# vnoz/Mutual-Information-MultiModal

Hardware: AMD Instinct MI355X
Metric: img-txt pairs/sec (MI critic fwd+bwd), global-batch InfoNCE (higher is better)
Workload: dtype bf16; 1 GPU; BASELINE configs[3]: global-batch infonce (reference semantics), bilinear critic fwd+bwd, B_global=4096, d=512; global_batch=4096, embed_dim=512, critic=bilinear, estimator=infonce, parallelism=single GPU, boundary=fp32 embeddings in, fp32 gradients out, hip_graph=False, graph_mode=none (direct C-ABI calls)

## Files before the change

mutual-information-multimodal_amd/csrc/mi_bilinear_flash.h:

```cpp
#pragma once
#include <type_traits>

#include "mi_common.h"

namespace mi {

#ifdef MI_STAMPS
#define MI_FL_STAMP(slot)                                                                       \
  do {                                                                                          \
    __builtin_amdgcn_sched_barrier(0);                                                          \
    if (threadIdx.x == 0 && g_stamps) g_stamps[(size_t)blockIdx.x * 16 + (slot)] = __builtin_amdgcn_s_memtime(); \
    __builtin_amdgcn_sched_barrier(0);                                                          \
  } while (0)
#else
#define MI_FL_STAMP(slot) do {} while (0)
#endif

#ifndef MI_FL_DIAG
#define MI_FL_DIAG 0
#endif
constexpr int kFlDiag = MI_FL_DIAG;
constexpr int kFlRows = 128;
constexpr int kFlBN = 32;
constexpr int kFlStages = 4;
constexpr float kFlThr = 60.0f;
constexpr int kFlMaxTilesPerSplit = 64;

struct FlashProblem {
  const bf16_t* q;
  const bf16_t* kv;
  const int64_t* sid_q;
  const int64_t* sid_kv;
  int64_t m, n;
  int64_t diag;
  int n_rb;
  int n_split;
  int tiles_per_split;
  const unsigned char* dup;
  float* slab;
  Partial* rec;
};
struct FlashArgs {
  FlashProblem p[2];
  int n_problems;
  int n_combo;
  int xcd_rows;
  int diag;
  int slab_f16;
  int no_index_mask;
};

template <int D>
struct FlashCfg {
  static constexpr int NK = D / 16;
  static constexpr int NT = D / 32;
  static constexpr int RB = D * 2;
  static constexpr int CPR = RB / 16;
  static constexpr int RPP = 1024 / RB;
  static constexpr int STAGE = kFlBN * RB;
  static constexpr int PIECES = STAGE / 1024 / 4;
  static constexpr int SID_OFF = kFlStages * STAGE;
  static constexpr size_t SMEM = (size_t)SID_OFF + (size_t)kFlMaxTilesPerSplit * kFlBN * 8;
  static constexpr int QA = NT >= 16 ? NK / 2 : 0;
  static constexpr int OA = NT >= 16 ? 12 : NT;
  static_assert(D == 128 || D == 256 || D == 512, "unsupported embedding width");
};

__host__ __device__ constexpr int fl_swz(int row) { return ((row & 3) << 2) | ((row >> 2) & 3); }

__device__ __forceinline__ float wave_max_uniform(float v) {
  int x;
#define MI_DPP_MAX(ctrl, rmask)                                                        \
  x = __builtin_amdgcn_update_dpp(__float_as_int(v), __float_as_int(v), ctrl, rmask, 0xF, false); \
  v = fmaxf(v, __int_as_float(x));
  MI_DPP_MAX(0xB1, 0xF)
  MI_DPP_MAX(0x4E, 0xF)
  MI_DPP_MAX(0x141, 0xF)
  MI_DPP_MAX(0x140, 0xF)
  MI_DPP_MAX(0x142, 0xA)
  MI_DPP_MAX(0x143, 0xC)
#undef MI_DPP_MAX
  return __int_as_float(__builtin_amdgcn_readlane(__float_as_int(v), 63));
}

__device__ __forceinline__ void fl_dma16(unsigned voff, const void* sbase, unsigned lds_addr) {
  unsigned keep;
  const uintptr_t b = (uintptr_t)sbase;
  const unsigned blo = __builtin_amdgcn_readfirstlane((unsigned)b), bhi = __builtin_amdgcn_readfirstlane((unsigned)(b >> 32));
  sbase = (const void*)(((uintptr_t)bhi << 32) | blo);
  lds_addr = __builtin_amdgcn_readfirstlane(lds_addr);
  asm volatile("s_mov_b32 %0, m0\n\ts_mov_b32 m0, %3\n\ts_nop 1\n\tglobal_load_lds_dwordx4 %1, %2\n\ts_mov_b32 m0, %0"
               : "=&s"(keep)
               : "v"(voff), "s"(sbase), "s"(lds_addr)
               : "memory");
}

template <int LOFF>
__device__ __forceinline__ void fl_dma_set_m0(unsigned lds_base) {
  asm volatile("s_add_u32 m0, %0, %1" : : "s"(lds_base), "n"(LOFF) : "scc");
}
template <int GOFF, int XORC>
__device__ __forceinline__ void fl_dma16_at(unsigned vlane_w, const void* sbase) {
  unsigned voff;
  asm volatile("v_xor_b32 %0, %3, %1\n\tglobal_load_lds_dwordx4 %0, %2 offset:%4"
               : "=&v"(voff)
               : "v"(vlane_w), "s"(sbase), "n"(XORC), "n"(GOFF)
               : "memory");
}

__device__ __forceinline__ float fl_max3(float a, float b, float c) {
  float d;
  asm("v_max3_f32 %0, %1, %2, %3" : "=v"(d) : "v"(a), "v"(b), "v"(c));
  return d;
}

__device__ __forceinline__ void fl_v_exp(const float& x) { asm volatile("v_exp_f32 %0, %0" : : "v"(x)); }
__device__ __forceinline__ void fl_v_add(const float& acc, const float& p) { asm volatile("v_add_f32 %0, %0, %1" : : "v"(acc), "v"(p)); }
__device__ __forceinline__ void fl_v_opaque(float& x) { asm volatile("; fl_opaque" : "+v"(x)); }
__device__ __forceinline__ unsigned fl_v_cvt_pk(const float& lo, const float& hi) {
  unsigned d;
  asm volatile("v_cvt_pk_bf16_f32 %0, %1, %2" : "=v"(d) : "v"(lo), "v"(hi));
  return d;
}
__device__ __forceinline__ void fl_v_prescale(float& x, const float& s, const float& off) {
  asm volatile("v_fmamk_f32 %0, %1, 0x3fb8aa3b, %2" : "=v"(x) : "v"(s), "v"(off));
}
__device__ __forceinline__ void fl_v_max(float& d, const float& a, const float& b) {
  asm volatile("v_max_f32 %0, %1, %2" : "=v"(d) : "v"(a), "v"(b));
}
__device__ __forceinline__ void fl_v_max3(float& d, const float& a, const float& b) {
  asm volatile("v_max3_f32 %0, %0, %1, %2" : "+v"(d) : "v"(a), "v"(b));
}
template <int STEP, bool NOP>
__device__ __forceinline__ void fl_dpp_max(const float& v) {
#define MI_FL_DPP(ctrl)                                                                            \
  if constexpr (NOP) asm volatile("s_nop 1\n\tv_max_f32_dpp %0, %0, %0 " ctrl : : "v"(v));          \
  else asm volatile("v_max_f32_dpp %0, %0, %0 " ctrl : : "v"(v))
  if constexpr (STEP == 0) { MI_FL_DPP("quad_perm:[1,0,3,2] row_mask:0xf bank_mask:0xf"); }
  else if constexpr (STEP == 1) { MI_FL_DPP("quad_perm:[2,3,0,1] row_mask:0xf bank_mask:0xf"); }
  else if constexpr (STEP == 2) { MI_FL_DPP("row_half_mirror row_mask:0xf bank_mask:0xf"); }
  else if constexpr (STEP == 3) { MI_FL_DPP("row_mirror row_mask:0xf bank_mask:0xf"); }
  else if constexpr (STEP == 4) { MI_FL_DPP("row_bcast:15 row_mask:0xa bank_mask:0xf"); }
  else { MI_FL_DPP("row_bcast:31 row_mask:0xc bank_mask:0xf"); }
#undef MI_FL_DPP
}

template <int N>
__device__ __forceinline__ void fl_wait_vmcnt_barrier() {
  asm volatile("s_waitcnt vmcnt(%0)\n\ts_barrier" ::"n"(N) : "memory");
}

template <int B, int E, class F>
__device__ __forceinline__ void fl_static_for(F&& f) {
  if constexpr (B < E) {
    f(std::integral_constant<int, B>{});
    fl_static_for<B + 1, E>(f);
  }
}

constexpr int kFlRing = 9;
constexpr int kFlAhead = 8;

template <int SLOT, int OFF>
__device__ __forceinline__ void fl_ring_read_s(bf16x8& f, int addr) {
  static_assert(OFF >= 0 && OFF < 65536, "ds offset field");
  if constexpr (SLOT == 0)
    asm volatile("ds_read_b128 v[216:219], %1 offset:%c2" : "={v[216:219]}"(f) : "v"(addr), "i"(OFF));
  else if constexpr (SLOT == 1)
    asm volatile("ds_read_b128 v[220:223], %1 offset:%c2" : "={v[220:223]}"(f) : "v"(addr), "i"(OFF));
  else if constexpr (SLOT == 2)
    asm volatile("ds_read_b128 v[224:227], %1 offset:%c2" : "={v[224:227]}"(f) : "v"(addr), "i"(OFF));
  else if constexpr (SLOT == 3)
    asm volatile("ds_read_b128 v[228:231], %1 offset:%c2" : "={v[228:231]}"(f) : "v"(addr), "i"(OFF));
  else if constexpr (SLOT == 4)
    asm volatile("ds_read_b128 v[232:235], %1 offset:%c2" : "={v[232:235]}"(f) : "v"(addr), "i"(OFF));
  else if constexpr (SLOT == 5)
    asm volatile("ds_read_b128 v[236:239], %1 offset:%c2" : "={v[236:239]}"(f) : "v"(addr), "i"(OFF));
  else if constexpr (SLOT == 6)
    asm volatile("ds_read_b128 v[240:243], %1 offset:%c2" : "={v[240:243]}"(f) : "v"(addr), "i"(OFF));
  else if constexpr (SLOT == 7)
    asm volatile("ds_read_b128 v[244:247], %1 offset:%c2" : "={v[244:247]}"(f) : "v"(addr), "i"(OFF));
  else if constexpr (SLOT == 8)
    asm volatile("ds_read_b128 v[248:251], %1 offset:%c2" : "={v[248:251]}"(f) : "v"(addr), "i"(OFF));
  else if constexpr (SLOT == 9)
    asm volatile("ds_read_b128 v[252:255], %1 offset:%c2" : "={v[252:255]}"(f) : "v"(addr), "i"(OFF));
}
template <int SLOT, int OFF_LO, int OFF_HI>
__device__ __forceinline__ void fl_ring_read_v(bf16x8& f, int addr_lo, int addr_hi) {
  static_assert(OFF_LO >= 0 && OFF_HI < 65536, "ds offset field");
  if constexpr (SLOT == 0)
    asm volatile("ds_read_b64_tr_b16 v[216:217], %1 offset:%c3\n\tds_read_b64_tr_b16 v[218:219], %2 offset:%c4"
                 : "={v[216:219]}"(f) : "v"(addr_lo), "v"(addr_hi), "i"(OFF_LO), "i"(OFF_HI));
  else if constexpr (SLOT == 1)
    asm volatile("ds_read_b64_tr_b16 v[220:221], %1 offset:%c3\n\tds_read_b64_tr_b16 v[222:223], %2 offset:%c4"
                 : "={v[220:223]}"(f) : "v"(addr_lo), "v"(addr_hi), "i"(OFF_LO), "i"(OFF_HI));
  else if constexpr (SLOT == 2)
    asm volatile("ds_read_b64_tr_b16 v[224:225], %1 offset:%c3\n\tds_read_b64_tr_b16 v[226:227], %2 offset:%c4"
                 : "={v[224:227]}"(f) : "v"(addr_lo), "v"(addr_hi), "i"(OFF_LO), "i"(OFF_HI));
  else if constexpr (SLOT == 3)
    asm volatile("ds_read_b64_tr_b16 v[228:229], %1 offset:%c3\n\tds_read_b64_tr_b16 v[230:231], %2 offset:%c4"
                 : "={v[228:231]}"(f) : "v"(addr_lo), "v"(addr_hi), "i"(OFF_LO), "i"(OFF_HI));
  else if constexpr (SLOT == 4)
    asm volatile("ds_read_b64_tr_b16 v[232:233], %1 offset:%c3\n\tds_read_b64_tr_b16 v[234:235], %2 offset:%c4"
                 : "={v[232:235]}"(f) : "v"(addr_lo), "v"(addr_hi), "i"(OFF_LO), "i"(OFF_HI));
  else if constexpr (SLOT == 5)
    asm volatile("ds_read_b64_tr_b16 v[236:237], %1 offset:%c3\n\tds_read_b64_tr_b16 v[238:239], %2 offset:%c4"
                 : "={v[236:239]}"(f) : "v"(addr_lo), "v"(addr_hi), "i"(OFF_LO), "i"(OFF_HI));
  else if constexpr (SLOT == 6)
    asm volatile("ds_read_b64_tr_b16 v[240:241], %1 offset:%c3\n\tds_read_b64_tr_b16 v[242:243], %2 offset:%c4"
                 : "={v[240:243]}"(f) : "v"(addr_lo), "v"(addr_hi), "i"(OFF_LO), "i"(OFF_HI));
  else if constexpr (SLOT == 7)
    asm volatile("ds_read_b64_tr_b16 v[244:245], %1 offset:%c3\n\tds_read_b64_tr_b16 v[246:247], %2 offset:%c4"
                 : "={v[244:247]}"(f) : "v"(addr_lo), "v"(addr_hi), "i"(OFF_LO), "i"(OFF_HI));
  else if constexpr (SLOT == 8)
    asm volatile("ds_read_b64_tr_b16 v[248:249], %1 offset:%c3\n\tds_read_b64_tr_b16 v[250:251], %2 offset:%c4"
                 : "={v[248:251]}"(f) : "v"(addr_lo), "v"(addr_hi), "i"(OFF_LO), "i"(OFF_HI));
  else if constexpr (SLOT == 9)
    asm volatile("ds_read_b64_tr_b16 v[252:253], %1 offset:%c3\n\tds_read_b64_tr_b16 v[254:255], %2 offset:%c4"
                 : "={v[252:255]}"(f) : "v"(addr_lo), "v"(addr_hi), "i"(OFF_LO), "i"(OFF_HI));
}
template <int WAIT>
__device__ __forceinline__ void fl_wait_lgkm() {
  if constexpr (kFlDiag & 16) return;
  if constexpr (WAIT >= 0) asm volatile("s_waitcnt lgkmcnt(%c0)" ::"i"(WAIT) : "memory");
}
template <bool B_IN_ACC, bool FIRST, int WAIT>
__device__ __forceinline__ void fl_mfma_s(f32x16& acc, const bf16x8& a, const bf16x8& b) {
  fl_wait_lgkm<WAIT>();
  if constexpr (FIRST) {
    if constexpr (B_IN_ACC)
      asm volatile("v_mfma_f32_32x32x16_bf16 %0, %1, %2, 0" : "=v"(acc) : "v"(a), "a"(b));
    else
      asm volatile("v_mfma_f32_32x32x16_bf16 %0, %1, %2, 0" : "=v"(acc) : "v"(a), "v"(b));
  } else {
    if constexpr (B_IN_ACC)
      asm volatile("v_mfma_f32_32x32x16_bf16 %0, %1, %2, %0" : : "v"(acc), "v"(a), "a"(b));
    else
      asm volatile("v_mfma_f32_32x32x16_bf16 %0, %1, %2, %0" : : "v"(acc), "v"(a), "v"(b));
  }
}
template <bool ACC_IN_ACC, bool NOP, int WAIT, class AT>
__device__ __forceinline__ void fl_mfma_o(f32x16& acc, const AT& a, const bf16x8& b) {
  static_assert(sizeof(AT) == 16, "a 32x32x16 bf16 operand is four registers");
  fl_wait_lgkm<WAIT>();
  if constexpr (NOP) {
    if constexpr (ACC_IN_ACC)
      asm volatile("s_nop 1\n\tv_mfma_f32_32x32x16_bf16 %0, %1, %2, %0" : "+a"(acc) : "v"(a), "v"(b));
    else
      asm volatile("s_nop 1\n\tv_mfma_f32_32x32x16_bf16 %0, %1, %2, %0" : "+v"(acc) : "v"(a), "v"(b));
  } else {
    if constexpr (ACC_IN_ACC)
      asm volatile("v_mfma_f32_32x32x16_bf16 %0, %1, %2, %0" : "+a"(acc) : "v"(a), "v"(b));
    else
      asm volatile("v_mfma_f32_32x32x16_bf16 %0, %1, %2, %0" : "+v"(acc) : "v"(a), "v"(b));
  }
}
template <bool DRAIN>
__device__ __forceinline__ void fl_score_fence(f32x16& acc) {
  if constexpr (DRAIN) asm volatile("s_nop 15\n\ts_nop 3" : "+v"(acc));
  else asm volatile("" : "+v"(acc));
}
__device__ __forceinline__ void fl_mfma_drain_all() { asm volatile("s_nop 15\n\ts_nop 3" ::: "memory"); }
template <bool IN_ACC>
__device__ __forceinline__ void fl_scale_tile(f32x16& t, float f) {
#pragma unroll
  for (int r = 0; r < 16; ++r) {
    if constexpr (IN_ACC) {
      float e = t[r], tmp;
      asm volatile("v_accvgpr_read_b32 %1, %0\n\tv_mul_f32 %1, %1, %2\n\tv_accvgpr_write_b32 %0, %1"
                   : "+a"(e), "=&v"(tmp)
                   : "v"(f));
      t[r] = e;
    } else {
      t[r] *= f;
    }
  }
}
template <bool IN_ACC>
__device__ __forceinline__ void fl_pin(bf16x8& v) {
  if constexpr (IN_ACC) asm volatile("" : "+a"(v));
  else asm volatile("" : "+v"(v));
}
template <bool IN_ACC>
__device__ __forceinline__ void fl_pin_o(f32x16& v) {
  if constexpr (IN_ACC) asm volatile("" : "+a"(v));
  else asm volatile("" : "+v"(v));
}

#ifndef MI_FL_WAIT_GROUP
#define MI_FL_WAIT_GROUP 2
#endif
constexpr int kFlWaitGroup = MI_FL_WAIT_GROUP;
template <int NS, int NV>
constexpr int fl_wait_count(int n) {
  if (n % kFlWaitGroup) return -1;
  int c = 0;
  for (int m = n + kFlWaitGroup; m <= n + kFlAhead - 1 && m < NS + NV; ++m) c += m < NS ? 1 : 2;
  return c;
}

template <int D, bool GRAD>
__global__ __launch_bounds__(256, 1) void bilinear_flash_kernel(FlashArgs args) {
  using C = FlashCfg<D>;
  extern __shared__ __attribute__((aligned(16))) char smem[];

  const FlashProblem A = args.p[0], Bp = args.p[1];
  const int n_combo = args.n_combo, n_problems = args.n_problems;
  asm volatile("" ::"s"(A.q), "s"(A.kv), "s"(A.sid_q), "s"(A.sid_kv), "s"(A.m), "s"(A.n), "s"(A.diag), "s"(A.n_rb),
               "s"(A.n_split), "s"(A.tiles_per_split), "s"(A.dup), "s"(A.slab), "s"(A.rec));
  asm volatile("" ::"s"(Bp.q), "s"(Bp.kv), "s"(Bp.sid_q), "s"(Bp.sid_kv), "s"(Bp.m), "s"(Bp.n), "s"(Bp.diag), "s"(Bp.n_rb),
               "s"(Bp.n_split), "s"(Bp.tiles_per_split), "s"(Bp.dup), "s"(Bp.slab), "s"(Bp.rec), "s"(n_combo),
               "s"(n_problems));
  const int L = (int)blockIdx.x;
  int prob, split, rb;
  if (args.xcd_rows) {
    const int ns_max = A.n_split > Bp.n_split ? A.n_split : Bp.n_split;
    const int x = L & 7, k = L >> 3;
    const int unit = x + 8 * (k / ns_max);
    split = k % ns_max;
    const int n_units = A.n_rb + (n_problems == 2 ? Bp.n_rb : 0);
    if (unit >= n_units) return;
    prob = unit >= A.n_rb ? 1 : 0;
    rb = prob ? unit - A.n_rb : unit;
    if (split >= (prob ? Bp.n_split : A.n_split)) return;
  } else {
    const int combo = L % n_combo;
    rb = L / n_combo;
    if (combo < A.n_split) {
      prob = 0;
      split = combo;
    } else if (n_problems == 2 && combo < A.n_split + Bp.n_split) {
      prob = 1;
      split = combo - A.n_split;
    } else {
      return;
    }
  }
  FlashProblem P;
  P.q = prob ? Bp.q : A.q;
  P.kv = prob ? Bp.kv : A.kv;
  P.sid_q = prob ? Bp.sid_q : A.sid_q;
  P.sid_kv = prob ? Bp.sid_kv : A.sid_kv;
  P.m = prob ? Bp.m : A.m;
  P.n = prob ? Bp.n : A.n;
  P.diag = prob ? Bp.diag : A.diag;
  P.n_rb = prob ? Bp.n_rb : A.n_rb;
  P.n_split = prob ? Bp.n_split : A.n_split;
  P.tiles_per_split = prob ? Bp.tiles_per_split : A.tiles_per_split;
  P.dup = prob ? Bp.dup : A.dup;
  P.slab = prob ? Bp.slab : A.slab;
  P.rec = prob ? Bp.rec : A.rec;
  if (rb >= P.n_rb) return;
  const int64_t n_tiles_all = P.n / kFlBN;
  const int64_t tile0 = (int64_t)split * P.tiles_per_split;
  int nt = (int)(n_tiles_all - tile0 < P.tiles_per_split ? n_tiles_all - tile0 : P.tiles_per_split);
  if (nt < 0) nt = 0;

  const int tid = threadIdx.x;
  const int wave = __builtin_amdgcn_readfirstlane(tid >> 6), lane = tid & 63;
  const int r32 = lane & 31, half = lane >> 5;
  const int64_t m_wave = (int64_t)rb * kFlRows + wave * 32;
  const bool wave_active = m_wave < P.m;
  const int64_t gi = wave_active ? m_wave + r32 : r32;
  MI_WALL_SCOPE(kWallFlash);
  MI_FL_STAMP(0);

  bf16x8 qf[C::NK];
  {
    const bf16_t* qblk = P.q + ((gi >> 5) * C::NK * 64 + lane) * 8;
#pragma unroll
    for (int kk = 0; kk < C::NK; ++kk) qf[kk] = *reinterpret_cast<const bf16x8*>(qblk + kk * 512);
  }
  const int64_t sid_i = P.sid_q[gi];
  MI_FL_STAMP(11);
  unsigned long long dupmask, diagmask;
  {
    const unsigned char* df = P.dup + (wave_active ? m_wave / 32 : 0) * n_tiles_all + tile0;
    const int flag = lane < nt ? (int)df[lane] : 0;
    dupmask = __ballot(flag == 2 || (flag == 1 && args.no_index_mask));
    diagmask = __ballot(flag == 1 && !args.no_index_mask);
  }

  const char* kv_base = reinterpret_cast<const char*>(P.kv + tile0 * kFlBN * D);
  const unsigned lds0 = (unsigned)(uintptr_t)(__attribute__((address_space(3))) char*)smem;
  const int lr = lane / C::CPR;
  const unsigned vlane = (unsigned)(lr * C::RB + 16 * ((lane % C::CPR) ^ (C::RPP > 1 ? (lr << 2) : 0)));
  auto piece_u = [](int q) __attribute__((always_inline)) {
    return C::RPP == 1 ? fl_swz(q) : (C::RPP == 2 ? (8 * (q & 1)) | ((q >> 1) & 3) : (q & 3));
  };
  const unsigned vlane_w = vlane ^ (unsigned)(16 * piece_u(C::PIECES * wave));
  auto piece_voff = [&](int i) __attribute__((always_inline)) { return vlane_w ^ (unsigned)(16 * piece_u(i)); };
  auto issue_piece = [&](int t, int i) __attribute__((always_inline)) {
    if ((kFlDiag & 1) && t >= 3) return;
    const int q = C::PIECES * wave + i;
    const int stage = t & (kFlStages - 1);
    fl_dma16(piece_voff(i), kv_base + (int64_t)t * C::STAGE + q * 1024, lds0 + stage * C::STAGE + q * 1024);
  };
  auto issue_tile = [&](int t) __attribute__((always_inline)) {
#pragma unroll
    for (int i = 0; i < C::PIECES; ++i) issue_piece(t, i);
  };
  MI_FL_STAMP(12);
  if (nt > 0) issue_tile(0);
  if (nt > 1) issue_tile(1);
  if (nt > 2) issue_tile(2);
  MI_FL_STAMP(13);

  {
    int64_t* sl = reinterpret_cast<int64_t*>(smem + C::SID_OFF);
    const int64_t* sg = P.sid_kv + tile0 * kFlBN;
    constexpr int PER = kFlMaxTilesPerSplit * kFlBN / 256;
    int64_t v[PER];
#pragma unroll
    for (int k = 0; k < PER; ++k) v[k] = tid + 256 * k < nt * kFlBN ? sg[tid + 256 * k] : 0;
#pragma unroll
    for (int k = 0; k < PER; ++k)
      if (tid + 256 * k < nt * kFlBN) sl[tid + 256 * k] = v[k];
  }

  constexpr int NO = GRAD ? C::NT : 1;
  f32x16 o[NO];
#pragma unroll
  for (int c = 0; c < NO; ++c)
#pragma unroll
    for (int r = 0; r < 16; ++r) o[c][r] = 0.0f;
  float lsum = 0.0f, pos = 0.0f;
  unsigned cnt = 0;
  float mref = MI_NEG_INF;

  const int fxh = half ^ fl_swz(r32);
  const int a0_lane = r32 * C::RB + 16 * fxh;
  const int g16 = lane >> 4, q4 = (lane & 15) >> 2, p4 = lane & 3;
  const int cl = 2 * (g16 & 1) + (p4 >> 1);
  const int a1_lane = (4 * half + q4) * C::RB + 16 * ((cl ^ half) | (q4 << 2)) + 8 * (p4 & 1);
  const int d0_wave = (int)(m_wave + P.diag - tile0 * kFlBN);

  MI_FL_STAMP(14);
  asm volatile("s_waitcnt vmcnt(0)" ::: "memory");
  MI_FL_STAMP(15);
  __syncthreads();
  MI_FL_STAMP(1);
  asm volatile("" ::"v"(sid_i), "s"(dupmask), "s"(diagmask));
  fl_static_for<0, C::NK>([&](auto KK) __attribute__((always_inline)) { fl_pin<(decltype(KK)::value < C::QA)>(qf[decltype(KK)::value]); });
  if constexpr (GRAD) fl_static_for<0, C::NT>([&](auto CT) __attribute__((always_inline)) { fl_pin_o<(decltype(CT)::value < C::OA)>(o[decltype(CT)::value]); });

  bf16x8 ring[kFlRing];
  u32x4 pfw[2];
  f32x16 s_next;
  float xs[16];
  float tA = MI_NEG_INF, tB = MI_NEG_INF, off = 0.0f;
  float f_pend = 1.0f;

  constexpr int kTailSlots = 17, kHeadSlots = 17;
  auto tail_slot = [&](auto S_) __attribute__((always_inline)) {
    constexpr int sl = decltype(S_)::value;
    if constexpr (kFlDiag & 2) return;
    if constexpr (sl < 16 && !(kFlDiag & 32)) fl_v_exp(xs[sl]);
    if constexpr (sl >= 1 && sl <= 16 && !(kFlDiag & 64)) fl_v_add(lsum, xs[sl - 1]);
    if constexpr (GRAD && sl >= 2 && sl <= 16 && sl % 2 == 0 && !(kFlDiag & 128)) {
      constexpr int k = sl / 2 - 1;
      pfw[k >> 2][k & 3] = fl_v_cvt_pk(xs[2 * k], xs[2 * k + 1]);
    }
  };
  auto decide = [&](const float& tmaxv, float thr) __attribute__((always_inline)) {
    float tmax_s, tmax_v, m_old;
    asm volatile(
        "s_nop 0\n\t"
        "v_readlane_b32 %[t], %[ta], 63\n\t"
        "v_mov_b32 %[mo], %[m]\n\t"
        "v_add_f32 %[f], %[th], %[m]\n\t"
        "v_mov_b32 %[tv], %[t]\n\t"
        "v_cmp_gt_f32 vcc, %[tv], %[f]\n\t"
        "v_sub_f32 %[f], %[m], %[tv]\n\t"
        "v_mul_f32 %[f], 0x3fb8aa3b, %[f]\n\t"
        "v_exp_f32 %[f], %[f]\n\t"
        "v_cndmask_b32 %[m], %[m], %[tv], vcc\n\t"
        "s_nop 0\n\t"
        "v_cndmask_b32 %[f], 1.0, %[f], vcc\n\t"
        "v_cmp_class_f32 vcc, %[mo], 4\n\t"
        "v_max_f32 %[o], 0xf149f2ca, %[m]\n\t"
        "v_mul_f32 %[o], 0xbfb8aa3b, %[o]\n\t"
        "v_cndmask_b32 %[f], %[f], 1.0, vcc"
        : [t] "=&s"(tmax_s), [tv] "=&v"(tmax_v), [mo] "=&v"(m_old), [f] "+v"(f_pend), [m] "+v"(mref),
          [o] "+v"(off)
        : [ta] "v"(tmaxv), [th] "s"(thr)
        : "vcc");
  };
  auto head_slot = [&](auto V_, auto NOPS_, float thr) __attribute__((always_inline)) {
    constexpr int v = decltype(V_)::value;
    constexpr bool NOPS = decltype(NOPS_)::value;
    if constexpr (kFlDiag & 2) return;
    if constexpr ((kFlDiag & 256) && v <= 10) return;
    if constexpr ((kFlDiag & 512) && v >= 11) return;
    if constexpr ((kFlDiag & 1024) && v <= 3) return;
    if constexpr ((kFlDiag & 2048) && v >= 4 && v <= 9) return;
    if constexpr ((kFlDiag & 4096) && v == 10) return;
    if constexpr (v == 0) {
      asm volatile("" : "+v"(s_next));
      cnt += 1024u;
      fl_v_max(tA, s_next[0], s_next[1]);
      fl_v_max(tB, s_next[2], s_next[3]);
    } else if constexpr (v >= 1 && v <= 3) {
      fl_v_max3(tA, s_next[4 * v], s_next[4 * v + 1]);
      fl_v_max3(tB, s_next[4 * v + 2], s_next[4 * v + 3]);
    } else if constexpr (v == 4) {
      fl_v_max(tA, tA, tB);
      fl_dpp_max<0, true>(tA);
    } else if constexpr (v >= 5 && v <= 9) {
      fl_dpp_max<v - 4, NOPS>(tA);
    } else if constexpr (v == 10) {
      decide(tA, thr);
    } else if constexpr (v >= 11 && v <= 14) {
      constexpr int r = 3 * (v - 11);
      fl_v_prescale(xs[r], s_next[r], off);
      fl_v_prescale(xs[r + 1], s_next[r + 1], off);
      fl_v_prescale(xs[r + 2], s_next[r + 2], off);
    } else if constexpr (v == 15 || v == 16) {
      constexpr int r = 12 + 2 * (v - 15);
      fl_v_prescale(xs[r], s_next[r], off);
      fl_v_prescale(xs[r + 1], s_next[r + 1], off);
    }
  };
  auto fix_masked_tile = [&](int tn) __attribute__((always_inline)) {
    unsigned mbits = 0u;
    float tq;
    unsigned long long m1;
    cnt -= 1024u;
    const int d0 = d0_wave - tn * kFlBN;
    const int want = r32 + d0 - 4 * half;
    const bool has_pos = want >= 0 && want < 32 && !(want & 4) && d0 > -32 && d0 < 32;
    const unsigned pbit = has_pos ? 1u << ((want & 3) + 4 * (want >> 3)) : 0u;
    if (__builtin_amdgcn_readfirstlane((int)((dupmask >> tn) & 1ull))) {
      MI_FL_STAMP(5);
      const int64_t* sl = reinterpret_cast<const int64_t*>(smem + C::SID_OFF) + tn * kFlBN + 4 * half;
#pragma unroll
      for (int r = 0; r < 16; ++r) {
        const bool neg = sl[(r & 3) + 8 * (r >> 2)] != sid_i;
        cnt += (unsigned)__popcll(__ballot(neg));
        mbits |= neg ? 0u : (1u << r);
        asm volatile("" : "+v"(mbits) : : "memory");
      }
      MI_FL_STAMP(6);
    } else {
      mbits = pbit;
      cnt += 1024u - 32u;
    }
    const float ninf = MI_NEG_INF;
    const float tmax_all = __int_as_float(__builtin_amdgcn_readlane(__float_as_int(tA), 63));
    const bool redo = __builtin_amdgcn_readfirstlane((int)(tmax_all > mref + kFlThr || mref == MI_NEG_INF)) != 0;
    if (!redo) {
#pragma unroll
      for (int r = 0; r < 16; r += 2) {
        unsigned t, u;
        const float s0 = s_next[r], s1 = s_next[r + 1];
        asm volatile("v_and_b32 %[t], %[b0], %[pb]\n\t"
                     "v_and_b32 %[u], %[b1], %[pb]\n\t"
                     "v_cmp_ne_u32 vcc, 0, %[t]\n\t"
                     "v_cmp_ne_u32 %[m1], 0, %[u]\n\t"
                     "v_and_b32 %[t], %[b0], %[mb]\n\t"
                     "v_and_b32 %[u], %[b1], %[mb]\n\t"
                     "v_cndmask_b32 %[q], 0, %[s0], vcc\n\t"
                     "v_add_f32 %[p], %[p], %[q]\n\t"
                     "v_cndmask_b32 %[q], 0, %[s1], %[m1]\n\t"
                     "v_add_f32 %[p], %[p], %[q]\n\t"
                     "v_cmp_ne_u32 vcc, 0, %[t]\n\t"
                     "v_cmp_ne_u32 %[m1], 0, %[u]\n\t"
                     "s_nop 1\n\t"
                     "v_cndmask_b32 %[x0], %[x0], %[ni], vcc\n\t"
                     "v_cndmask_b32 %[x1], %[x1], %[ni], %[m1]"
                     : [t] "=&v"(t), [u] "=&v"(u), [q] "=&v"(tq), [m1] "=&s"(m1), [p] "+v"(pos), [x0] "+v"(xs[r]), [x1] "+v"(xs[r + 1])
                     : [b0] "n"(1 << r), [b1] "n"(2 << r), [mb] "v"(mbits), [pb] "v"(pbit), [s0] "v"(s0), [s1] "v"(s1), [ni] "v"(ninf)
                     : "vcc");
      }
      return;
    }
    float tM = MI_NEG_INF;
#pragma unroll
    for (int r = 0; r < 16; ++r) {
      unsigned t;
      const float sr = s_next[r];
      asm volatile("v_and_b32 %[t], %[b], %[mb]\n\t"
                   "v_cmp_eq_u32 vcc, 0, %[t]\n\t"
                   "s_nop 1\n\t"
                   "v_cndmask_b32 %[t], %[ni], %[s], vcc\n\t"
                   "v_max_f32 %[tm], %[tm], %[t]\n\t"
                   "v_and_b32 %[t], %[b], %[pb]\n\t"
                   "v_cmp_ne_u32 vcc, 0, %[t]\n\t"
                   "s_nop 1\n\t"
                   "v_cndmask_b32 %[t], 0, %[s], vcc\n\t"
                   "v_add_f32 %[p], %[p], %[t]"
                   : [t] "=&v"(t), [tm] "+v"(tM), [p] "+v"(pos)
                   : [b] "n"(1 << r), [mb] "v"(mbits), [pb] "v"(pbit), [s] "v"(sr), [ni] "v"(ninf)
                   : "vcc");
    }
    float tmaxv = wave_max_uniform(tM);
    asm volatile("s_nop 1" : "+v"(tmaxv));
    decide(tmaxv, kFlThr);
#pragma unroll
    for (int r = 0; r < 16; ++r) {
      unsigned t;
      const float sr = s_next[r];
      asm volatile("v_fmamk_f32 %[x], %[s], 0x3fb8aa3b, %[o]\n\t"
                   "v_and_b32 %[t], %[b], %[mb]\n\t"
                   "v_cmp_eq_u32 vcc, 0, %[t]\n\t"
                   "s_nop 1\n\t"
                   "v_cndmask_b32 %[x], %[ni], %[x], vcc"
                   : [x] "+v"(xs[r]), [t] "=&v"(t)
                   : [b] "n"(1 << r), [mb] "v"(mbits), [s] "v"(sr), [o] "v"(off), [ni] "v"(ninf)
                   : "vcc");
    }
  };

  const unsigned long long spmask = dupmask | diagmask;

  auto iteration = [&](auto HAS_S_, auto HAS_V_, int tp) __attribute__((always_inline)) {
    constexpr bool HAS_S = decltype(HAS_S_)::value, HAS_V = decltype(HAS_V_)::value && GRAD;
    constexpr bool DO_TAIL = decltype(HAS_V_)::value;
    constexpr int NS = HAS_S ? C::NK : 0, NV = HAS_V ? 2 * C::NT : 0, NF = NS + NV;
    const bool masked_next = __builtin_amdgcn_readfirstlane((int)((spmask >> ((tp + 1) & 63)) & 1ull)) != 0;
    const float thr_next = masked_next ? __builtin_inff() : kFlThr;
    fl_v_opaque(lsum);
    if constexpr (DO_TAIL && !(kFlDiag & 2)) {
      if (__builtin_expect(__builtin_amdgcn_readfirstlane((int)__float_as_uint(f_pend)) != 0x3f800000, 0)) {
        lsum *= f_pend;
        fl_v_opaque(lsum);
        if constexpr (GRAD) {
          fl_mfma_drain_all();
          fl_static_for<0, C::NT>([&](auto CT) __attribute__((always_inline)) { fl_scale_tile<(decltype(CT)::value < C::OA)>(o[decltype(CT)::value], f_pend); });
        }
        f_pend = 1.0f;
        fl_v_opaque(f_pend);
      }
    }
    const int so = ((tp + 1) & (kFlStages - 1)) * C::STAGE + a0_lane;
    const int vo = (tp & (kFlStages - 1)) * C::STAGE + a1_lane;
    int abase[8], tbase[8];
    if constexpr (HAS_S) {
#pragma unroll
      for (int v = 0; v < 8; ++v) abase[v] = so ^ (32 * v);
    }
    if constexpr (HAS_V) {
#pragma unroll
      for (int v = 0; v < 8; ++v) tbase[v] = vo ^ (16 * ((4 * (v >> 1)) ^ (2 * (v & 1))));
    }
    auto issue_read = [&](auto NI) __attribute__((always_inline)) {
      constexpr int n = decltype(NI)::value;
      if constexpr (kFlDiag & 8) return;
      if constexpr (n < NS) {
        fl_ring_read_s<n % kFlRing, 256 * (n >> 3)>(ring[n % kFlRing], abase[n & 7]);
      } else if constexpr (n < NF) {
        constexpr int u = n - NS, ks = u / C::NT, ct = u % C::NT;
        fl_ring_read_v<n % kFlRing, 256 * (ct >> 2) + 16 * ks * C::RB, 256 * (ct >> 2) + (16 * ks + 8) * C::RB>(
            ring[n % kFlRing], tbase[2 * (ct & 3)], tbase[2 * (ct & 3) + 1]);
      }
    };
    fl_static_for<0, kFlAhead>([&](auto NI) __attribute__((always_inline)) { issue_read(NI); });
    __builtin_amdgcn_sched_barrier(0);
    fl_static_for<0, NS>([&](auto NI) __attribute__((always_inline)) {
      constexpr int n = decltype(NI)::value;
      fl_mfma_s<(n < C::QA), n == 0, fl_wait_count<NS, NV>(n)>(s_next, ring[n % kFlRing], qf[n]);
      issue_read(std::integral_constant<int, n + kFlAhead>{});
      if constexpr (DO_TAIL) {
        constexpr int NSD = NS > 0 ? NS : 1;
        constexpr int per = (kTailSlots + NSD - 1) / NSD;
        constexpr int lo = n * per, hi = (lo + per < kTailSlots ? lo + per : kTailSlots);
        fl_static_for<(lo < kTailSlots ? lo : kTailSlots), hi>([&](auto SI) __attribute__((always_inline)) { tail_slot(SI); });
      }
      __builtin_amdgcn_sched_barrier(0);
    });
    if constexpr (DO_TAIL && !HAS_S) {
      fl_static_for<0, kTailSlots>([&](auto SI) __attribute__((always_inline)) { tail_slot(SI); });
      __builtin_amdgcn_sched_barrier(0);
    }
    if constexpr (HAS_S && !HAS_V) {
      fl_score_fence<true>(s_next);
      fl_static_for<0, kHeadSlots>([&](auto VI) __attribute__((always_inline)) { head_slot(VI, std::true_type{}, thr_next); });
      __builtin_amdgcn_sched_barrier(0);
    }
    if constexpr (HAS_V) {
      constexpr int EVERY = NV / C::PIECES;
      const int tq = tp + 3 < nt ? tp + 3 : nt - 1;
      const uintptr_t gb = (uintptr_t)(kv_base + (int64_t)tq * C::STAGE + wave * (C::PIECES * 1024));
      const unsigned gb_lo = __builtin_amdgcn_readfirstlane((unsigned)gb);
      const unsigned gb_hi = __builtin_amdgcn_readfirstlane((unsigned)(gb >> 32));
      const void* sb0 = (const void*)(((uintptr_t)gb_hi << 32) | gb_lo);
      const void* sb1 = (const char*)sb0 + 4096;
      const unsigned lb = __builtin_amdgcn_readfirstlane(lds0 + (unsigned)(((tp + 3) & (kFlStages - 1)) * C::STAGE) +
                                                         (unsigned)(wave * (C::PIECES * 1024)));
      constexpr int U0 = 5;
      constexpr int n_avail = (NV - U0) - (NV / EVERY - U0 / EVERY);
      static_assert(n_avail >= 1, "no gap for the softmax head");
      fl_static_for<0, NV>([&](auto UI) __attribute__((always_inline)) {
        constexpr int u = decltype(UI)::value, n = NS + u, ks = u / C::NT, ct = u % C::NT;
        fl_mfma_o<(ct < C::OA), (u % C::NT == 0), fl_wait_count<NS, NV>(n)>(o[ct], pfw[ks], ring[n % kFlRing]);
        issue_read(std::integral_constant<int, n + kFlAhead>{});
        constexpr bool dma_gap = u % EVERY == EVERY - 1;
        if constexpr (HAS_S && u >= U0 && !dma_gap) {
          constexpr int k = (u - U0) - (u / EVERY - U0 / EVERY);
          constexpr int lo = k * kHeadSlots / n_avail, hi = (k + 1) * kHeadSlots / n_avail;
          constexpr bool nops = kHeadSlots > n_avail;
          fl_static_for<lo, hi>([&](auto VI) __attribute__((always_inline)) { head_slot(VI, std::integral_constant<bool, nops>{}, thr_next); });
        }
        if constexpr (HAS_S && !(kFlDiag & 1) && u % EVERY == EVERY - 3 && ((u / EVERY) & 3) == 0 && u / EVERY < C::PIECES)
          fl_dma_set_m0<((u / EVERY) & ~3) * 1024>(lb);
        if constexpr (dma_gap && HAS_S && !(kFlDiag & 1)) {
          constexpr int i = u / EVERY;
          fl_dma16_at<(i & 3) * 1024,
                      16 * (C::RPP == 1 ? fl_swz(i) : (C::RPP == 2 ? (8 * (i & 1)) | ((i >> 1) & 3) : (i & 3)))>(
              vlane_w, i < 4 ? sb0 : sb1);
        }
        __builtin_amdgcn_sched_barrier(0);
      });
    } else if constexpr (DO_TAIL) {
      if (tp + 3 < nt) issue_tile(tp + 3);
    }
    if constexpr (HAS_S && !(kFlDiag & 2)) {
      if (__builtin_expect(masked_next, 0)) fix_masked_tile(tp + 1);
    }
  };
  using T_ = std::true_type;
  using F_ = std::false_type;

  if (nt > 0) {
    iteration(T_{}, F_{}, -1);
    for (int t = 0; t + 1 < nt; ++t) {
      if (t == nt / 2) MI_FL_STAMP(2);
      if constexpr (kFlDiag & 4) asm volatile("s_waitcnt vmcnt(0)" ::: "memory");
      else if constexpr (GRAD) fl_wait_vmcnt_barrier<C::PIECES>();
      else if (t + 2 < nt) fl_wait_vmcnt_barrier<C::PIECES>();
      else fl_wait_vmcnt_barrier<0>();
      if (t == nt / 2) MI_FL_STAMP(3);
      iteration(T_{}, T_{}, t);
      if (t == nt / 2) MI_FL_STAMP(4);
    }
    MI_FL_STAMP(8);
    iteration(F_{}, T_{}, nt - 1);
  }
  MI_FL_STAMP(9);

  fl_v_opaque(lsum);
  lsum = wave_sum(lsum);
  pos = wave_sum(pos);
  if (lane == 0) {
    Partial rec{mref, lsum, pos, cnt};
    if (!wave_active) rec = Partial{MI_NEG_INF, 0.0f, 0.0f, 0u};
    seam_store<kSeam_FLASH>(&P.rec[((int64_t)split * P.n_rb + rb) * 4 + wave], rec);
  }
  if constexpr (GRAD) {
    fl_mfma_drain_all();
    fl_static_for<0, C::NT>([&](auto CT) __attribute__((always_inline)) { fl_pin_o<(decltype(CT)::value < C::OA)>(o[decltype(CT)::value]); });
    const int64_t wv = ((int64_t)split * P.n_rb + rb) * 4 + wave;
    if (wave_active && args.slab_f16) {
      float amax = 0.0f;
#pragma unroll
      for (int c = 0; c < C::NT; ++c)
#pragma unroll
        for (int r = 0; r < 16; ++r) amax = fmaxf(amax, __builtin_fabsf(o[c][r]));
      amax = wave_max_uniform(amax);
      int k = 13 - ((int)((__float_as_uint(amax) >> 23) & 255u) - 127);
      k = amax > 0.0f ? (k < -100 ? -100 : (k > 100 ? 100 : k)) : 0;
      const float up = __uint_as_float((unsigned)(127 + k) << 23), down = __uint_as_float((unsigned)(127 - k) << 23);
      f16_t* slab16 = reinterpret_cast<f16_t*>(P.slab);
      float* unscale = reinterpret_cast<float*>(slab16 + (int64_t)P.n_split * P.n_rb * 4 * (32 * D));
      if (lane == 0) seam_store<kSeam_FLASH>(&unscale[wv], down);
      f16_t* dst = slab16 + wv * (32 * D) + lane * 8;
#pragma unroll
      for (int c = 0; c < C::NT; ++c)
#pragma unroll
        for (int gp = 0; gp < 2; ++gp) {
          f16x8 h;
#pragma unroll
          for (int e = 0; e < 8; ++e) h[e] = (f16_t)(o[c][8 * gp + e] * up);
          seam_store<kSeam_FLASH>(reinterpret_cast<f16x8*>(dst + c * 1024 + gp * 512), h);
        }
    } else if (wave_active) {
      float* dst = P.slab + wv * (32 * D) + lane * 4;
#pragma unroll
      for (int c = 0; c < C::NT; ++c)
#pragma unroll
        for (int g = 0; g < 4; ++g) {
          const f32x4 v = {o[c][4 * g], o[c][4 * g + 1], o[c][4 * g + 2], o[c][4 * g + 3]};
          seam_store<kSeam_FLASH>(reinterpret_cast<f32x4*>(dst + c * 1024 + g * 256), v);
        }
    }
  }
  MI_FL_STAMP(10);
}

static __global__ __launch_bounds__(256) void flash_dup_flags_kernel(const int64_t* __restrict__ sid_rows,
                                                                     const int64_t* __restrict__ sid_cols, int na, int nb,
                                                                     unsigned char* __restrict__ flag,
                                                                     unsigned char* __restrict__ flag_t) {
  __shared__ int64_t rows[32];
  const int a = blockIdx.x, tid = threadIdx.x;
  if (tid < 32) rows[tid] = sid_rows[a * 32 + tid];
  __syncthreads();
  const int q = tid & 3;
  int64_t mine[8];
#pragma unroll
  for (int e = 0; e < 8; ++e) mine[e] = rows[8 * q + e];
  for (int b = blockIdx.y * 64 + (tid >> 2); b < nb; b += gridDim.y * 64) {
    const int64_t* c = sid_cols + (int64_t)b * 32;
    bool any = false;
    for (int j = 0; j < 32; ++j) {
      const int64_t v = c[j];
#pragma unroll
      for (int e = 0; e < 8; ++e) any |= v == mine[e];
    }
    int f = any ? 1 : 0;
    f |= __shfl_xor(f, 1);
    f |= __shfl_xor(f, 2);
    if (q == 0) {
      flag[(int64_t)a * nb + b] = (unsigned char)f;
      flag_t[(int64_t)b * na + a] = (unsigned char)f;
    }
  }
}

static inline int launch_flash_dup_flags(const int64_t* sid_rows, const int64_t* sid_cols, int64_t br, int64_t b,
                                         unsigned char* flag, unsigned char* flag_t, hipStream_t st) {
  const int na = (int)(br / 32), nb = (int)(b / 32);
  int gy = (nb + 63) / 64;
  if (gy > 8) gy = 8;
  {
    ProfScope prof_("bilinear equal-id tile flags", st);
    hipLaunchKernelGGL(flash_dup_flags_kernel, dim3((unsigned)na, (unsigned)gy), dim3(256), 0, st, sid_rows, sid_cols, na, nb,
                       flag, flag_t);
  }
  MI_LAUNCH_CHECK("flash_dup_flags_kernel");
  return MI_OK;
}

struct FlashReduceJob {
  const float* slab;
  const Partial* rec;
  int n_split, n_rb;
  int64_t m;
  const bf16_t* other;
  int64_t n_other, diag;
  float* out_f32;
  bf16_t* out_bf;
  bf16_t* out_bf_t;
};
struct FlashReduceArgs {
  FlashReduceJob j[2];
  const mi_stats* stats;
  const float* grad_out;
};

template <int D, bool F16>
__global__ __launch_bounds__(256) void flash_reduce_kernel(FlashReduceArgs args) {
  kernarg_prefetch<(int)sizeof(FlashReduceArgs)>();
  __shared__ float tile[32][129];
  const FlashReduceJob& J = args.j[blockIdx.z];
  const int64_t wb = blockIdx.y;
  const int cc = blockIdx.x;
  if (wb * 32 >= J.m) return;
  const int rb = (int)(wb >> 2), w = (int)(wb & 3);
  const float go = args.grad_out ? args.grad_out[0] : 1.0f;
  const float lse = args.stats->lse;
  const float gpos = go / (float)args.stats->n_pos;
  const int tid = threadIdx.x;
  float acc[16];
#pragma unroll
  for (int e = 0; e < 16; ++e) acc[e] = 0.0f;
  const int64_t i0 = wb * 32;
  const int64_t c0 = (int64_t)cc * 128;
  const int orow = tid >> 3, ocs = (tid & 7) * 16;
  const int64_t ojo = i0 + orow + J.diag;
  const bool has_other = ojo >= 0 && ojo < J.n_other;
  bf16x8 oth_a = {}, oth_b = {};
  if (has_other) {
    oth_a = *reinterpret_cast<const bf16x8*>(J.other + ojo * D + c0 + ocs);
    oth_b = *reinterpret_cast<const bf16x8*>(J.other + ojo * D + c0 + ocs + 8);
  }
  const f16_t* slab16 = reinterpret_cast<const f16_t*>(J.slab);
  const float* unscale = reinterpret_cast<const float*>(slab16 + (int64_t)J.n_split * J.n_rb * 4 * (32 * D));
  for (int s0 = 0; s0 < J.n_split; s0 += 4) {
    float cs[4];
    int64_t wvs[4];
#pragma unroll
    for (int q = 0; q < 4; ++q) {
      const int s = s0 + q < J.n_split ? s0 + q : J.n_split - 1;
      wvs[q] = ((int64_t)s * J.n_rb + rb) * 4 + w;
      const float m = J.rec[wvs[q]].m;
      cs[q] = (s0 + q < J.n_split && m > MI_NEG_INF) ? go * __expf(m - lse) * (F16 ? unscale[wvs[q]] : 1.0f) : 0.0f;
    }
    if constexpr (F16) {
      f16x8 v[4][2];
#pragma unroll
      for (int q = 0; q < 4; ++q)
#pragma unroll
        for (int u = 0; u < 2; ++u)
          v[q][u] = *reinterpret_cast<const f16x8*>(slab16 + wvs[q] * (32 * D) + (int64_t)cc * 4096 + (u * 256 + tid) * 8);
#pragma unroll
      for (int q = 0; q < 4; ++q)
        if (cs[q] != 0.0f) {
#pragma unroll
          for (int u = 0; u < 2; ++u)
#pragma unroll
            for (int e = 0; e < 8; ++e) acc[8 * u + e] += (float)v[q][u][e] * cs[q];
        }
    } else {
      f32x4 v[4][4];
#pragma unroll
      for (int q = 0; q < 4; ++q)
#pragma unroll
        for (int u = 0; u < 4; ++u)
          v[q][u] = *reinterpret_cast<const f32x4*>(J.slab + wvs[q] * (32 * D) + (int64_t)cc * 4096 + (u * 256 + tid) * 4);
#pragma unroll
      for (int q = 0; q < 4; ++q)
        if (cs[q] != 0.0f) {
#pragma unroll
          for (int u = 0; u < 4; ++u)
#pragma unroll
            for (int e = 0; e < 4; ++e) acc[4 * u + e] += v[q][u][e] * cs[q];
        }
    }
  }
  if constexpr (F16) {
#pragma unroll
    for (int u = 0; u < 2; ++u) {
      const int h = u * 256 + tid;
      const int ct_l = h >> 7, gp = (h >> 6) & 1, lane = h & 63;
      const int col = ct_l * 32 + (lane & 31);
#pragma unroll
      for (int hh = 0; hh < 2; ++hh) {
        const int row0 = 8 * (2 * gp + hh) + 4 * (lane >> 5);
#pragma unroll
        for (int e = 0; e < 4; ++e) tile[row0 + e][col] = acc[8 * u + 4 * hh + e];
      }
    }
  } else {
#pragma unroll
    for (int u = 0; u < 4; ++u) {
      const int f = u * 256 + tid;
      const int ct_l = f >> 8, g = (f >> 6) & 3, lane = f & 63;
      const int col = ct_l * 32 + (lane & 31), row0 = 8 * g + 4 * (lane >> 5);
#pragma unroll
      for (int e = 0; e < 4; ++e) tile[row0 + e][col] = acc[4 * u + e];
    }
  }
  __syncthreads();
  {
    const int row = orow, cs = ocs;
    const int64_t i = i0 + row;
    float v[16];
#pragma unroll
    for (int e = 0; e < 16; ++e) v[e] = tile[row][cs + e];
    if (has_other) {
#pragma unroll
      for (int e = 0; e < 8; ++e) {
        v[e] -= gpos * (float)oth_a[e];
        v[8 + e] -= gpos * (float)oth_b[e];
      }
#pragma unroll
      for (int e = 0; e < 16; ++e) tile[row][cs + e] = v[e];
    }
    if (J.out_f32) {
#pragma unroll
      for (int e = 0; e < 16; e += 4)
        *reinterpret_cast<f32x4*>(J.out_f32 + i * D + c0 + cs + e) = f32x4{v[e], v[e + 1], v[e + 2], v[e + 3]};
    }
    if (J.out_bf) {
      bf16x8 a, b;
#pragma unroll
      for (int e = 0; e < 8; ++e) {
        a[e] = (bf16_t)v[e];
        b[e] = (bf16_t)v[8 + e];
      }
      *reinterpret_cast<bf16x8*>(J.out_bf + i * D + c0 + cs) = a;
      *reinterpret_cast<bf16x8*>(J.out_bf + i * D + c0 + cs + 8) = b;
    }
  }
  if (J.out_bf_t) {
    __syncthreads();
    const int col = tid >> 1, rs = (tid & 1) * 16;
    bf16x8 a, b;
#pragma unroll
    for (int e = 0; e < 8; ++e) {
      a[e] = (bf16_t)tile[rs + e][col];
      b[e] = (bf16_t)tile[rs + 8 + e][col];
    }
    bf16_t* dst = J.out_bf_t + (c0 + col) * J.m + i0 + rs;
    *reinterpret_cast<bf16x8*>(dst) = a;
    *reinterpret_cast<bf16x8*>(dst + 8) = b;
  }
}

struct FlashPlan {
  bool ok;
  int n_split[2], n_rb[2], tiles_per_split[2];
  int64_t slab_bytes[2], n_rec[2];
  bool slab_f16;
};

static inline bool flash_width_ok(int64_t d) { return d == 128 || d == 256 || d == 512; }

static inline FlashPlan flash_plan(int64_t br, int64_t b, int64_t d) {
  FlashPlan fp{};
  static const bool off = getenv("MI_NO_FLASH") != nullptr;
  fp.ok = !off && flash_width_ok(d) && br % 32 == 0 && b % 32 == 0 && br >= 32;
  if (!fp.ok) return fp;
  static const bool slab_f32 = getenv("MI_FLASH_SLAB_F32") != nullptr;
  fp.slab_f16 = !slab_f32;
  const int64_t m[2] = {br, b}, n[2] = {b, br};
  int64_t total_tiles = 0;
  for (int q = 0; q < 2; ++q) {
    fp.n_rb[q] = (int)((m[q] + kFlRows - 1) / kFlRows);
    total_tiles += (int64_t)fp.n_rb[q] * (n[q] / kFlBN);
  }
  int64_t tau = (total_tiles + 255) / 256;
  if (tau < 4) tau = 4;
  if (tau > kFlMaxTilesPerSplit) tau = kFlMaxTilesPerSplit;
  if (const char* e = getenv("MI_FLASH_TILES")) tau = atoi(e) > 0 ? atoi(e) : tau;
  for (int q = 0; q < 2; ++q) {
    const int64_t tiles = n[q] / kFlBN;
    int64_t tps = tau < tiles ? tau : tiles;
    fp.n_split[q] = (int)((tiles + tps - 1) / tps);
    fp.tiles_per_split[q] = (int)((tiles + fp.n_split[q] - 1) / fp.n_split[q]);
// ... 65 lines not shown
```

Before: 41.23 million pairs/s.

## Skip DPP max reduction in pipelined head, redo tile only when max exceeds threshold

The pipelined softmax head no longer runs the full cross-lane DPP max reduction. Each lane instead compares its per-row max against a running limit (mref + threshold) and sets a raise mask, and only when some lane exceeds the limit does the tile get redone through the combined masked/raise slow path. The change also hoists the sid_kv global loads ahead of the initial DMA issue and relaxes the prologue wait to let two tiles stay in flight. This cuts VALU/DPP work in the steady-state loop at the cost of a divergent slow path on tiles where the max rises.

```diff
diff --git a/mutual-information-multimodal_amd/csrc/mi_bilinear_flash.h b/mutual-information-multimodal_amd/csrc/mi_bilinear_flash.h
--- a/mutual-information-multimodal_amd/csrc/mi_bilinear_flash.h
+++ b/mutual-information-multimodal_amd/csrc/mi_bilinear_flash.h
@@ -130,6 +130,9 @@
 }
 __device__ __forceinline__ void fl_v_max3(float& d, const float& a, const float& b) {
   asm volatile("v_max3_f32 %0, %0, %1, %2" : "+v"(d) : "v"(a), "v"(b));
+}
+__device__ __forceinline__ void fl_v_cmp_raise(unsigned long long& m, const float& tmax, const float& lim) {
+  asm volatile("v_cmp_gt_f32 %0, %1, %2" : "=s"(m) : "v"(tmax), "v"(lim));
 }
 template <int STEP, bool NOP>
 __device__ __forceinline__ void fl_dpp_max(const float& v) {
@@ -372,6 +375,13 @@
     for (int kk = 0; kk < C::NK; ++kk) qf[kk] = *reinterpret_cast<const bf16x8*>(qblk + kk * 512);
   }
   const int64_t sid_i = P.sid_q[gi];
+  constexpr int kSidPer = kFlMaxTilesPerSplit * kFlBN / 256;
+  int64_t sidv[kSidPer];
+  {
+    const int64_t* sg = P.sid_kv + tile0 * kFlBN;
+#pragma unroll
+    for (int k = 0; k < kSidPer; ++k) sidv[k] = tid + 256 * k < nt * kFlBN ? sg[tid + 256 * k] : 0;
+  }
   MI_FL_STAMP(11);
   unsigned long long dupmask, diagmask;
   {
@@ -408,14 +418,9 @@
 
   {
     int64_t* sl = reinterpret_cast<int64_t*>(smem + C::SID_OFF);
-    const int64_t* sg = P.sid_kv + tile0 * kFlBN;
-    constexpr int PER = kFlMaxTilesPerSplit * kFlBN / 256;
-    int64_t v[PER];
-#pragma unroll
-    for (int k = 0; k < PER; ++k) v[k] = tid + 256 * k < nt * kFlBN ? sg[tid + 256 * k] : 0;
-#pragma unroll
-    for (int k = 0; k < PER; ++k)
-      if (tid + 256 * k < nt * kFlBN) sl[tid + 256 * k] = v[k];
+#pragma unroll
+    for (int k = 0; k < kSidPer; ++k)
+      if (tid + 256 * k < nt * kFlBN) sl[tid + 256 * k] = sidv[k];
   }
 
   constexpr int NO = GRAD ? C::NT : 1;
@@ -436,7 +441,8 @@
   const int d0_wave = (int)(m_wave + P.diag - tile0 * kFlBN);
 
   MI_FL_STAMP(14);
-  asm volatile("s_waitcnt vmcnt(0)" ::: "memory");
+  if (nt > 2) asm volatile("s_waitcnt vmcnt(%0)" ::"n"(2 * C::PIECES) : "memory");
+  else asm volatile("s_waitcnt vmcnt(0)" ::: "memory");
   MI_FL_STAMP(15);
   __syncthreads();
   MI_FL_STAMP(1);
@@ -450,8 +456,10 @@
   float xs[16];
   float tA = MI_NEG_INF, tB = MI_NEG_INF, off = 0.0f;
   float f_pend = 1.0f;
-
-  constexpr int kTailSlots = 17, kHeadSlots = 17;
+  float lim = MI_NEG_INF;
+  unsigned long long raise_mask = 0ull;
+
+  constexpr int kTailSlots = 17, kHeadSlots = 17, kPipeHeadSlots = 11;
   auto tail_slot = [&](auto S_) __attribute__((always_inline)) {
     constexpr int sl = decltype(S_)::value;
     if constexpr (kFlDiag & 2) return;
@@ -480,15 +488,17 @@
         "v_cmp_class_f32 vcc, %[mo], 4\n\t"
         "v_max_f32 %[o], 0xf149f2ca, %[m]\n\t"
         "v_mul_f32 %[o], 0xbfb8aa3b, %[o]\n\t"
-        "v_cndmask_b32 %[f], %[f], 1.0, vcc"
+        "v_cndmask_b32 %[f], %[f], 1.0, vcc\n\t"
+        "v_add_f32 %[l], %[kt], %[m]"
         : [t] "=&s"(tmax_s), [tv] "=&v"(tmax_v), [mo] "=&v"(m_old), [f] "+v"(f_pend), [m] "+v"(mref),
-          [o] "+v"(off)
-        : [ta] "v"(tmaxv), [th] "s"(thr)
+          [o] "+v"(off),
+          [l] "+v"(lim)
+        : [ta] "v"(tmaxv), [th] "s"(thr), [kt] "s"(kFlThr)
         : "vcc");
   };
-  auto head_slot = [&](auto V_, auto NOPS_, float thr) __attribute__((always_inline)) {
+  auto head_slot = [&](auto V_, auto NOPS_, auto INLINE_, float thr) __attribute__((always_inline)) {
     constexpr int v = decltype(V_)::value;
-    constexpr bool NOPS = decltype(NOPS_)::value;
+    constexpr bool NOPS = decltype(NOPS_)::value, INLINE = decltype(INLINE_)::value;
     if constexpr (kFlDiag & 2) return;
     if constexpr ((kFlDiag & 256) && v <= 10) return;
     if constexpr ((kFlDiag & 512) && v >= 11) return;
@@ -505,7 +515,8 @@
       fl_v_max3(tB, s_next[4 * v + 2], s_next[4 * v + 3]);
     } else if constexpr (v == 4) {
       fl_v_max(tA, tA, tB);
-      fl_dpp_max<0, true>(tA);
+      fl_v_cmp_raise(raise_mask, tA, lim);
+      if constexpr (INLINE) fl_dpp_max<0, true>(tA);
     } else if constexpr (v >= 5 && v <= 9) {
       fl_dpp_max<v - 4, NOPS>(tA);
     } else if constexpr (v == 10) {
@@ -521,79 +532,79 @@
       fl_v_prescale(xs[r + 1], s_next[r + 1], off);
     }
   };
-  auto fix_masked_tile = [&](int tn) __attribute__((always_inline)) {
+  auto redo_tile = [&](int tn, bool masked, bool raise_all) __attribute__((always_inline)) {
     unsigned mbits = 0u;
-    float tq;
-    unsigned long long m1;
-    cnt -= 1024u;
-    const int d0 = d0_wave - tn * kFlBN;
-    const int want = r32 + d0 - 4 * half;
-    const bool has_pos = want >= 0 && want < 32 && !(want & 4) && d0 > -32 && d0 < 32;
-    const unsigned pbit = has_pos ? 1u << ((want & 3) + 4 * (want >> 3)) : 0u;
-    if (__builtin_amdgcn_readfirstlane((int)((dupmask >> tn) & 1ull))) {
-      MI_FL_STAMP(5);
-      const int64_t* sl = reinterpret_cast<const int64_t*>(smem + C::SID_OFF) + tn * kFlBN + 4 * half;
+    const float ninf = MI_NEG_INF;
+    if (masked) {
+      float tq;
+      unsigned long long m1;
+      cnt -= 1024u;
+      const int d0 = d0_wave - tn * kFlBN;
+      const int want = r32 + d0 - 4 * half;
+      const bool has_pos = want >= 0 && want < 32 && !(want & 4) && d0 > -32 && d0 < 32;
+      const unsigned pbit = has_pos ? 1u << ((want & 3) + 4 * (want >> 3)) : 0u;
+      if (__builtin_amdgcn_readfirstlane((int)((dupmask >> tn) & 1ull))) {
+        MI_FL_STAMP(5);
+        const int64_t* sl = reinterpret_cast<const int64_t*>(smem + C::SID_OFF) + tn * kFlBN + 4 * half;
+#pragma unroll
+        for (int r = 0; r < 16; ++r) {
+          const bool neg = sl[(r & 3) + 8 * (r >> 2)] != sid_i;
+          cnt += (unsigned)__popcll(__ballot(neg));
+          mbits |= neg ? 0u : (1u << r);
+          asm volatile("" : "+v"(mbits) : : "memory");
+        }
+        MI_FL_STAMP(6);
+      } else {
+        mbits = pbit;
+        cnt += 1024u - 32u;
+      }
+      if (!raise_all) {
+#pragma unroll
+        for (int r = 0; r < 16; r += 2) {
+          unsigned t, u;
+          const float s0 = s_next[r], s1 = s_next[r + 1];
+          asm volatile("v_and_b32 %[t], %[b0], %[pb]\n\t"
+                       "v_and_b32 %[u], %[b1], %[pb]\n\t"
+                       "v_cmp_ne_u32 vcc, 0, %[t]\n\t"
+                       "v_cmp_ne_u32 %[m1], 0, %[u]\n\t"
+                       "v_and_b32 %[t], %[b0], %[mb]\n\t"
+                       "v_and_b32 %[u], %[b1], %[mb]\n\t"
+                       "v_cndmask_b32 %[q], 0, %[s0], vcc\n\t"
+                       "v_add_f32 %[p], %[p], %[q]\n\t"
+                       "v_cndmask_b32 %[q], 0, %[s1], %[m1]\n\t"
+                       "v_add_f32 %[p], %[p], %[q]\n\t"
+                       "v_cmp_ne_u32 vcc, 0, %[t]\n\t"
+                       "v_cmp_ne_u32 %[m1], 0, %[u]\n\t"
+                       "s_nop 1\n\t"
+                       "v_cndmask_b32 %[x0], %[x0], %[ni], vcc\n\t"
+                       "v_cndmask_b32 %[x1], %[x1], %[ni], %[m1]"
+                       : [t] "=&v"(t), [u] "=&v"(u), [q] "=&v"(tq), [m1] "=&s"(m1), [p] "+v"(pos), [x0] "+v"(xs[r]), [x1] "+v"(xs[r + 1])
+                       : [b0] "n"(1 << r), [b1] "n"(2 << r), [mb] "v"(mbits), [pb] "v"(pbit), [s0] "v"(s0), [s1] "v"(s1), [ni] "v"(ninf)
+                       : "vcc");
+        }
+        return;
+      }
+      asm volatile("v_mov_b32 %0, %1" : "+v"(tA) : "v"(ninf));
 #pragma unroll
       for (int r = 0; r < 16; ++r) {
-        const bool neg = sl[(r & 3) + 8 * (r >> 2)] != sid_i;
-        cnt += (unsigned)__popcll(__ballot(neg));
-        mbits |= neg ? 0u : (1u << r);
-        asm volatile("" : "+v"(mbits) : : "memory");
-      }
-      MI_FL_STAMP(6);
-    } else {
-      mbits = pbit;
-      cnt += 1024u - 32u;
-    }
-    const float ninf = MI_NEG_INF;
-    const float tmax_all = __int_as_float(__builtin_amdgcn_readlane(__float_as_int(tA), 63));
-    const bool redo = __builtin_amdgcn_readfirstlane((int)(tmax_all > mref + kFlThr || mref == MI_NEG_INF)) != 0;
-    if (!redo) {
-#pragma unroll
-      for (int r = 0; r < 16; r += 2) {
-        unsigned t, u;
-        const float s0 = s_next[r], s1 = s_next[r + 1];
-        asm volatile("v_and_b32 %[t], %[b0], %[pb]\n\t"
-                     "v_and_b32 %[u], %[b1], %[pb]\n\t"
+        unsigned t;
+        const float sr = s_next[r];
+        asm volatile("v_and_b32 %[t], %[b], %[mb]\n\t"
+                     "v_cmp_eq_u32 vcc, 0, %[t]\n\t"
+                     "s_nop 1\n\t"
+                     "v_cndmask_b32 %[t], %[ni], %[s], vcc\n\t"
+                     "v_max_f32 %[tm], %[tm], %[t]\n\t"
+                     "v_and_b32 %[t], %[b], %[pb]\n\t"
                      "v_cmp_ne_u32 vcc, 0, %[t]\n\t"
-                     "v_cmp_ne_u32 %[m1], 0, %[u]\n\t"
-                     "v_and_b32 %[t], %[b0], %[mb]\n\t"
-                     "v_and_b32 %[u], %[b1], %[mb]\n\t"
-                     "v_cndmask_b32 %[q], 0, %[s0], vcc\n\t"
-                     "v_add_f32 %[p], %[p], %[q]\n\t"
-                     "v_cndmask_b32 %[q], 0, %[s1], %[m1]\n\t"
-                     "v_add_f32 %[p], %[p], %[q]\n\t"
-                     "v_cmp_ne_u32 vcc, 0, %[t]\n\t"
-                     "v_cmp_ne_u32 %[m1], 0, %[u]\n\t"
                      "s_nop 1\n\t"
-                     "v_cndmask_b32 %[x0], %[x0], %[ni], vcc\n\t"
-                     "v_cndmask_b32 %[x1], %[x1], %[ni], %[m1]"
-                     : [t] "=&v"(t), [u] "=&v"(u), [q] "=&v"(tq), [m1] "=&s"(m1), [p] "+v"(pos), [x0] "+v"(xs[r]), [x1] "+v"(xs[r + 1])
-                     : [b0] "n"(1 << r), [b1] "n"(2 << r), [mb] "v"(mbits), [pb] "v"(pbit), [s0] "v"(s0), [s1] "v"(s1), [ni] "v"(ninf)
+                     "v_cndmask_b32 %[t], 0, %[s], vcc\n\t"
+                     "v_add_f32 %[p], %[p], %[t]"
+                     : [t] "=&v"(t), [tm] "+v"(tA), [p] "+v"(pos)
+                     : [b] "n"(1 << r), [mb] "v"(mbits), [pb] "v"(pbit), [s] "v"(sr), [ni] "v"(ninf)
                      : "vcc");
       }
-      return;
-    }
-    float tM = MI_NEG_INF;
-#pragma unroll
-    for (int r = 0; r < 16; ++r) {
-      unsigned t;
-      const float sr = s_next[r];
-      asm volatile("v_and_b32 %[t], %[b], %[mb]\n\t"
-                   "v_cmp_eq_u32 vcc, 0, %[t]\n\t"
-                   "s_nop 1\n\t"
-                   "v_cndmask_b32 %[t], %[ni], %[s], vcc\n\t"
-                   "v_max_f32 %[tm], %[tm], %[t]\n\t"
-                   "v_and_b32 %[t], %[b], %[pb]\n\t"
-                   "v_cmp_ne_u32 vcc, 0, %[t]\n\t"
-                   "s_nop 1\n\t"
-                   "v_cndmask_b32 %[t], 0, %[s], vcc\n\t"
-                   "v_add_f32 %[p], %[p], %[t]"
-                   : [t] "=&v"(t), [tm] "+v"(tM), [p] "+v"(pos)
-                   : [b] "n"(1 << r), [mb] "v"(mbits), [pb] "v"(pbit), [s] "v"(sr), [ni] "v"(ninf)
-                   : "vcc");
-    }
-    float tmaxv = wave_max_uniform(tM);
+    }
+    float tmaxv = wave_max_uniform(tA);
     asm volatile("s_nop 1" : "+v"(tmaxv));
     decide(tmaxv, kFlThr);
 #pragma unroll
@@ -674,7 +685,7 @@
     }
     if constexpr (HAS_S && !HAS_V) {
       fl_score_fence<true>(s_next);
-      fl_static_for<0, kHeadSlots>([&](auto VI) __attribute__((always_inline)) { head_slot(VI, std::true_type{}, thr_next); });
+      fl_static_for<0, kHeadSlots>([&](auto VI) __attribute__((always_inline)) { head_slot(VI, std::true_type{}, std::true_type{}, thr_next); });
       __builtin_amdgcn_sched_barrier(0);
     }
     if constexpr (HAS_V) {
@@ -697,9 +708,11 @@
         constexpr bool dma_gap = u % EVERY == EVERY - 1;
         if constexpr (HAS_S && u >= U0 && !dma_gap) {
           constexpr int k = (u - U0) - (u / EVERY - U0 / EVERY);
-          constexpr int lo = k * kHeadSlots / n_avail, hi = (k + 1) * kHeadSlots / n_avail;
-          constexpr bool nops = kHeadSlots > n_avail;
-          fl_static_for<lo, hi>([&](auto VI) __attribute__((always_inline)) { head_slot(VI, std::integral_constant<bool, nops>{}, thr_next); });
+          constexpr int lo = k * kPipeHeadSlots / n_avail, hi = (k + 1) * kPipeHeadSlots / n_avail;
+          fl_static_for<lo, hi>([&](auto PI) __attribute__((always_inline)) {
+            constexpr int p = decltype(PI)::value;
+            head_slot(std::integral_constant<int, (p <= 4 ? p : p + 6)>{}, std::false_type{}, std::false_type{}, thr_next);
+          });
         }
         if constexpr (HAS_S && !(kFlDiag & 1) && u % EVERY == EVERY - 3 && ((u / EVERY) & 3) == 0 && u / EVERY < C::PIECES)
           fl_dma_set_m0<((u / EVERY) & ~3) * 1024>(lb);
@@ -715,7 +728,9 @@
       if (tp + 3 < nt) issue_tile(tp + 3);
     }
     if constexpr (HAS_S && !(kFlDiag & 2)) {
-      if (__builtin_expect(masked_next, 0)) fix_masked_tile(tp + 1);
+      asm volatile("" : "+s"(raise_mask));
+      const bool raised = raise_mask != 0ull;
+      if (__builtin_expect(masked_next || (HAS_V && raised), 0)) redo_tile(tp + 1, masked_next, raised);
     }
   };
   using T_ = std::true_type;
```

After: 41.19 million pairs/s. About the same (-0.1%).
